# feldroop/floxer

Hardware: NVIDIA B200
Metric: pex_verification_gcups (higher is better)
Workload: dtype u32

## Files before the change

floxer_b200/csrc/dp_kernels.cuh:

```cuda
#pragma once

#include <cstdint>
#include <cuda_runtime.h>

namespace fxg {

constexpr int kNumSymbols = 6;
constexpr int kPeqFrontPadWords = 64;
constexpr int kPeqBackPadWords = 66;
constexpr uint32_t kFlagReverse = 1u;
constexpr uint32_t kFlagInlineRef = 2u;
constexpr int32_t kNoScore = 0x3fffffff;
constexpr int32_t kPoisonScore = 0x7ffffff0;
constexpr uint32_t kWinChunks = 8;
constexpr uint32_t kWinBytes = 2 * kWinChunks * 32;

struct DpTask {
    uint64_t ref_base;
    uint64_t query_base;
    uint64_t trace_base;
    uint32_t n;
    uint32_t m;
    int32_t dlo, dhi;
    uint32_t flags;
// ... 344 lines not shown
        for (uint32_t c = r; c < fill; c += G) load_window_chunk(packed, store_chunks, first_chunk, reverse, c, win);
        uint32_t const n_words = nb * W;
        for (uint32_t w = r; w < n_words; w += G) {
            int32_t const virt = int32_t(pad) - int32_t(32 * w);
            uint32_t const wild = virt >= 32 ? 0xffffffffu : (virt > 0 ? ((1u << virt) - 1u) : 0u);
            uint32_t* const dst = peq + (w / W) * (kNumSymbols * W) + (w % W);
#pragma unroll
            for (int s = 0; s < kNumSymbols; ++s) {
                const uint32_t* plane = L.peq_table + uint64_t(s) * L.peq_plane_words;
                uint32_t x;
                if (!reverse) {
                    x = peq_window(plane, int64_t(T.query_base) - int64_t(pad) + int64_t(32 * w));
                } else {
                    int64_t const y = int64_t(T.query_base) + int64_t(T.m) - 1 + int64_t(pad) - int64_t(32 * w);
                    x = __brev(peq_window(plane, y - 31));
                }
                dst[s * W] = x | wild;
            }
        }
    }
    __syncwarp();

    uint32_t const last_block = nb - 1;
    uint32_t const ck_per_block = ck_records_per_block(int64_t(T.dhi) - int64_t(T.dlo) + 1, ROWS);
    LaneState<W> S;
    S.acc_hp = 0; S.acc_hn = 0; S.ckp = nullptr;
#pragma unroll
    for (int i = 0; i < W; ++i) { S.Pv[i] = 0; S.Mv[i] = 0; }
    S.b = r; S.o_hp = 0x80000000u; S.o_hn = 0;
    S.score = 0; S.best = kNoScore; S.best_col = 0;
    S.eqb = peq;
    int32_t ce_up = 0;
    auto set_block = [&](uint32_t blk) {
        S.cs = 0x7fffffff; S.ce = -1;
        if (!have_task || blk >= nb) return;
        {
            int32_t const hi_up = int32_t(ROWS) * int32_t(blk) + dhi;
            ce_up = hi_up > int32_t(T.n) ? int32_t(T.n) : hi_up;
        }
        int32_t const lo = int32_t(ROWS) * int32_t(blk) + 1 + dlo;
        int32_t const hi = int32_t(ROWS) * int32_t(blk + 1) + dhi;
        int32_t const cs = lo < 1 ? 1 : lo;
        int32_t const ce = hi > int32_t(T.n) ? int32_t(T.n) : hi;
        if (cs <= ce) { S.cs = cs; S.ce = ce; }
    };
    set_block(S.b);
    uint32_t const src_lane = in_ring ? slot * G + (r + G - 1) % G : lane;

    uint32_t const my_end = __reduce_max_sync(0xffffffffu, have_task ? (T.n + nb - 1) : 0u);
    constexpr uint32_t kNever = 0x7fffffffu;

    auto flush_boundary_bits = [&](uint32_t t) {
        uint32_t const left_over = (t - 1) & 31u;
        if (left_over) {
            uint32_t const hb = __brev(S.acc_hp) >> (32 - left_over), nbits = __brev(S.acc_hn) >> (32 - left_over);
            if constexpr (W == 1) *reinterpret_cast<uint2*>(S.ckp + 2) = make_uint2(hb, nbits);
            else *reinterpret_cast<uint4*>(S.ckp + 2 * W) = make_uint4(hb, nbits, 0u, 0u);
        }
    };

    uint32_t my_refill = 0;
    uint32_t t = 1;
    while (t <= my_end) {
        uint32_t const r_hp = __shfl_sync(0xffffffffu, S.o_hp, src_lane);
        uint32_t const r_hn = __shfl_sync(0xffffffffu, S.o_hn, src_lane);
        int32_t const r_sc = __shfl_sync(0xffffffffu, S.score, src_lane);
        if (S.ce >= 0 && int32_t(t) - int32_t(S.b) > S.ce) {
            if (CKPT) flush_boundary_bits(t);
            S.b += G; set_block(S.b);
        }
        int32_t const j = int32_t(t) - int32_t(S.b);
        if (j == S.cs) {
#pragma unroll
            for (int i = 0; i < W; ++i) { S.Pv[i] = 0xffffffffu; S.Mv[i] = 0; }
            if (S.b == 0) {
#pragma unroll
                for (int i = 0; i < W; ++i) {
                    int32_t const virt = int32_t(pad) - 32 * i;
                    S.Pv[i] = virt >= 32 ? 0u : (virt > 0 ? (0xffffffffu << virt) : 0xffffffffu);
                }
                S.score = int32_t(ROWS) - int32_t(pad);
            } else if (S.cs - 1 == ce_up) {
                S.score = r_sc + ROWS;
            } else {
                S.score = r_sc - int32_t(r_hp >> 31) + int32_t(r_hn >> 31) + ROWS;
            }
            S.eqb = peq + S.b * (kNumSymbols * W);
            if (CKPT) {
                S.acc_hp = 0xffffffffu; S.acc_hn = 0;
                S.ckp = L.trace + T.trace_base + uint64_t(S.b) * ck_per_block * ck_record_words(W);
            }
        }
        bool const active = j >= S.cs && j <= S.ce && !dead;
        if (__any_sync(0xffffffffu, t >= my_refill)) {
            my_refill = kNever;
            uint32_t new_base = c_base;
            uint32_t i_hi = 0;
            bool reading = false;
            if (have_task && !dead) {
                int32_t const ti = int32_t(t);
                int32_t const e1 = ti - int32_t(T.n);
                int32_t const e2n = ti - dhi - ROWS;
                int32_t const e2 = e2n > 0 ? (e2n + ROWS) / (ROWS + 1) : 0;
                int32_t const b_top = e1 > e2 ? e1 : e2;
                int32_t const s1 = ti - 1 - dlo;
                int32_t b_low = s1 > 0 ? s1 / (ROWS + 1) : 0;
                if (b_low > ti - 1) b_low = ti - 1;
                if (b_low > int32_t(last_block)) b_low = int32_t(last_block);
                reading = b_top <= int32_t(last_block);
                if (reading) {
                    i_hi = uint32_t(int32_t(phase) + ti + 1 - b_top);
                    if (i_hi >= 32 * (c_base + kWinChunks)) {
                        int32_t const lo = ti - 3 - b_low;
                        new_base = uint32_t(int32_t(phase) + (lo > 0 ? lo : 0)) >> 5;
                        if (new_base <= c_base || i_hi >= 32 * (new_base + kWinChunks)) { dead = true; new_base = c_base; }
                    }
                }
            }
            uint32_t const rounds = __reduce_max_sync(0xffffffffu, (new_base - c_base + G - 1) / G);
            for (uint32_t k = 0; k < rounds; ++k) {
                uint32_t const c = c_base + kWinChunks + r + k * G;
                if (c < new_base + kWinChunks) load_window_chunk(packed, store_chunks, first_chunk, reverse, c, win);
            }
            c_base = new_base;
            if (reading && !dead) my_refill = t + (32 * (c_base + kWinChunks) - i_hi);
        }
        __syncwarp();
        uint8_t const* const win0 = win + phase - 32 * kWinChunks * (c_base / kWinChunks);
        uint32_t my_evt = active ? uint32_t(S.ce) + S.b + 1u : (S.cs == 0x7fffffff ? kNever : uint32_t(S.cs) + S.b);
        my_evt = min(my_evt, my_refill);
        auto upper_at = [&](uint32_t step) {
            if (S.b == 0) return Upper{0u, 0u};
            return int32_t(step) - int32_t(S.b) > ce_up ? Upper{0u, 0x80000000u} : Upper{1u, 0u};
        };
        Upper const up_first = upper_at(t), up_rest = upper_at(t + 1);
        bool const peel = __any_sync(0xffffffffu, up_first.keep != up_rest.keep);
        if (active && S.b > 0 && int32_t(t) - int32_t(S.b) < ce_up) my_evt = min(my_evt, uint32_t(ce_up) + S.b);
        uint32_t const evt = min(__reduce_min_sync(0xffffffffu, my_evt), my_end + 1);
        bool const any_last = __any_sync(0xffffffffu, active && S.b == last_block);
        if (any_last) run_steps<W, CKPT, true>(S, t, evt, active, src_lane, last_block, win0, win, L.two, up_first, up_rest, peel);
        else run_steps<W, CKPT, false>(S, t, evt, active, src_lane, last_block, win0, win, L.two, up_first, up_rest, peel);
        t = evt;
    }
    if (CKPT && S.ce >= 0 && int32_t(t) - int32_t(S.b) > S.ce) flush_boundary_bits(t);
    uint32_t const owner = last_block % G;
    if (have_task && r == owner) {
        DpResult res; res.score = dead ? kPoisonScore : S.best; res.end_col = S.best_col;
        L.results[T.out] = res;
    }
}

__host__ __device__ constexpr int dp_min_ctas(int W) { return W <= 2 ? 28 : (W == 4 ? 25 : (W == 8 ? 19 : (W == 16 ? 14 : 8))); }
template <int W, bool CKPT>
__global__ void __launch_bounds__(32, dp_min_ctas(W)) dp_kernel(DpLaunch const L) {
    extern __shared__ __align__(16) uint8_t smem[];
    uint32_t const tasks_per_warp = 32u / L.group;
    uint32_t const n_tasks = L.n_tasks_dev ? __ldg(L.n_tasks_dev) : L.n_tasks;
    const DpTask* tasks = L.tasks;
    if (L.class_active) { for (uint32_t c = 0; c < L.cls; ++c) tasks += __ldg(L.class_active + c); }
    for (uint32_t g = blockIdx.x; g * tasks_per_warp < n_tasks; g += gridDim.x) {
        dp_task_group<W, CKPT>(L, tasks, g, n_tasks, smem);
        __syncwarp();
    }
}

constexpr uint32_t kWideThreads = 128;
constexpr uint32_t kWideG = 64;
__host__ __device__ constexpr size_t wide_smem_bytes() { return size_t(kNumSymbols) * 32 * kWideThreads * 4 + 2 * kWideThreads * 16; }

template <bool CKPT>
__global__ void __launch_bounds__(kWideThreads, 1) dp_wide_kernel(DpLaunch const L) {
    extern __shared__ __align__(16) uint8_t smem[];
    constexpr int W = 32;
    constexpr int ROWS = 32 * W;
    uint32_t* const eq_all = reinterpret_cast<uint32_t*>(smem);
    uint4* const pub = reinterpret_cast<uint4*>(smem + size_t(kNumSymbols) * 32 * kWideThreads * 4);
    uint32_t const l = threadIdx.x;
    uint32_t const n_tasks = L.n_tasks_dev ? __ldg(L.n_tasks_dev) : L.n_tasks;
    const DpTask* tasks = L.tasks;
    if (L.class_active) { for (uint32_t c = 0; c < L.cls; ++c) tasks += __ldg(L.class_active + c); }
    for (uint32_t task_id = blockIdx.x; task_id < n_tasks; task_id += gridDim.x) {
        DpTask const T = tasks[task_id];
        uint32_t const nb = (T.m + ROWS - 1) / ROWS;
        uint32_t const pad = nb * ROWS - T.m;
        int32_t const dlo = T.dlo - int32_t(pad), dhi = T.dhi - int32_t(pad);
        bool const reverse = (T.flags & kFlagReverse) != 0;
        const uint32_t* const packed = (T.flags & kFlagInlineRef) ? L.inline_packed : L.ref_packed;
        bool const have = l < nb;
        int32_t cs = 0x7fffffff, ce = -1;
        if (have) {
            int32_t const lo = int32_t(ROWS) * int32_t(l) + 1 + dlo, hi = int32_t(ROWS) * int32_t(l + 1) + dhi;
            int32_t const a = lo < 1 ? 1 : lo, b = hi > int32_t(T.n) ? int32_t(T.n) : hi;
            if (a <= b) { cs = a; ce = b; }
        }
        if (have) {
            for (int w = 0; w < W; ++w) {
                uint32_t const gw = l * W + uint32_t(w);
                int32_t const virt = int32_t(pad) - int32_t(32 * gw);
                uint32_t const wild = virt >= 32 ? 0xffffffffu : (virt > 0 ? ((1u << virt) - 1u) : 0u);
                for (int sym = 0; sym < kNumSymbols; ++sym) {
                    const uint32_t* plane = L.peq_table + uint64_t(sym) * L.peq_plane_words;
                    uint32_t x;
                    if (!reverse) x = peq_window(plane, int64_t(T.query_base) - int64_t(pad) + int64_t(32 * gw));
                    else x = __brev(peq_window(plane, int64_t(T.query_base) + int64_t(T.m) - 1 + int64_t(pad) - int64_t(32 * gw) - 31));
                    eq_all[(uint32_t(sym) * 32 + uint32_t(w)) * kWideThreads + l] = x | wild;
                }
            }
        }
        uint32_t Pv[W], Mv[W];
#pragma unroll
        for (int i = 0; i < W; ++i) { Pv[i] = 0; Mv[i] = 0; }
        int32_t score = 0, best = kNoScore;
        uint32_t best_col = 0;
        uint32_t acc_hp = 0xffffffffu, acc_hn = 0;
        uint32_t const ck_per_block = ck_records_per_block(int64_t(T.dhi) - int64_t(T.dlo) + 1, ROWS);
        uint32_t* ckp = CKPT ? L.trace + T.trace_base + uint64_t(l) * ck_per_block * ck_record_words(W) : nullptr;
        pub[l] = make_uint4(0x80000000u, 0u, 0u, 0u);
        pub[kWideThreads + l] = make_uint4(0x80000000u, 0u, 0u, 0u);
        __syncthreads();
        uint32_t const t_end = T.n + nb - 1;
        bool const is_last = have && l == nb - 1;
        for (uint32_t t = 1; t <= t_end; ++t) {
            int32_t const j = int32_t(t) - int32_t(l);
            uint4 const up = l > 0 ? pub[((t - 1) & 1u) * kWideThreads + l - 1] : make_uint4(0u, 0u, 0u, 0u);
            bool const active = have && j >= cs && j <= ce;
            uint4 mine = make_uint4(0x80000000u, 0u, uint32_t(score), 0u);
            if (active) {
                if (j == cs) {
#pragma unroll
                    for (int i = 0; i < W; ++i) { Pv[i] = 0xffffffffu; Mv[i] = 0; }
                    if (l == 0) {
#pragma unroll
                        for (int i = 0; i < W; ++i) {
                            int32_t const virt = int32_t(pad) - 32 * i;
                            Pv[i] = virt >= 32 ? 0u : (virt > 0 ? (0xffffffffu << virt) : 0xffffffffu);
                        }
                        score = int32_t(ROWS) - int32_t(pad);
                    } else if (cs - 1 == (int32_t(ROWS) * int32_t(l) + dhi > int32_t(T.n) ? int32_t(T.n) : int32_t(ROWS) * int32_t(l) + dhi)) {
                        score = int32_t(up.z) + ROWS;
                    } else {
                        score = int32_t(up.z) - int32_t(up.x >> 31) + int32_t(up.y >> 31) + ROWS;
                    }
                    acc_hp = 0xffffffffu; acc_hn = 0;
                }
                uint64_t const pos = reverse ? T.ref_base + uint64_t(T.n) - uint64_t(j) : T.ref_base + uint64_t(j) - 1;
                uint32_t c = packed_base(packed, pos);
                if (c >= uint32_t(kNumSymbols)) c = 0;
                uint32_t Eq[W];
#pragma unroll
                for (int w = 0; w < W; ++w) Eq[w] = eq_all[(c * 32 + uint32_t(w)) * kWideThreads + l];
                uint32_t hp, hn, no_hp[1];
                block_column<W, false>(Pv, Mv, Eq, l == 0 ? 0u : up.x, l == 0 ? 0u : up.y, hp, hn, no_hp);
                score += int32_t(hp >> 31) - int32_t(hn >> 31);
                if (is_last && score <= best) { best = score; best_col = uint32_t(j); }
                mine = make_uint4(hp, hn, uint32_t(score), 0u);
                if (CKPT) {
                    acc_hp = __funnelshift_l(hp, acc_hp, 1); acc_hn = __funnelshift_l(hn, acc_hn, 1);
                    if ((t & 31u) == 0) { write_checkpoint<W>(ckp, Pv, Mv, __brev(acc_hp), __brev(acc_hn)); ckp += ck_record_words(W); }
                    else if (j == ce) {
                        uint32_t const left_over = t & 31u;
                        *reinterpret_cast<uint4*>(ckp + 2 * W) = make_uint4(__brev(acc_hp) >> (32 - left_over), __brev(acc_hn) >> (32 - left_over), 0u, 0u);
                    }
                }
            }
            pub[(t & 1u) * kWideThreads + l] = mine;
            __syncthreads();
        }
        if (is_last) { DpResult res; res.score = best; res.end_col = best_col; L.results[T.out] = res; }
        __syncthreads();
    }
}

struct WalkResult {
    uint32_t begin_col;
    uint32_t cigar_len;
};

struct Walk2Task {
    uint64_t ck_base;
    uint64_t ref_base;
    uint64_t query_base;
    uint64_t cigar_base;
    uint32_t n, m;
    int32_t dlo, dhi;
    uint32_t end_col;
    uint32_t score;
    uint32_t flags;
    uint32_t cigar_cap;
    uint32_t out;
    uint32_t reserved;
};

struct Walk2Launch {
    const Walk2Task* tasks; uint32_t n_tasks;
    const uint32_t* ck;
    const uint32_t* ref_packed; const uint32_t* inline_packed;
    const uint32_t* peq_table; uint64_t peq_plane_words;
    const uint8_t* query_pool;
    uint32_t* cigars;
    WalkResult* results;
    uint32_t two;
};

__host__ __device__ constexpr uint32_t walk2_threads() { return 64u; }
__host__ __device__ constexpr uint32_t walk2_per_cta(uint32_t W) { return walk2_threads() / W; }
__host__ __device__ constexpr uint32_t walk2_words_per_group(uint32_t W) { return 64 * W + 2 + kNumSymbols * W + 8; }
__host__ __device__ constexpr size_t walk2_smem_bytes(uint32_t W) { return size_t(walk2_words_per_group(W)) * walk2_per_cta(W) * 4; }

template <int W>
__global__ void __launch_bounds__(walk2_threads()) walk2_kernel(Walk2Launch const L) {
    extern __shared__ __align__(16) uint32_t w2_smem[];
    constexpr int ROWS = 32 * W;
    constexpr uint32_t RECW = ck_record_words(W);
    constexpr uint32_t PER_CTA = walk2_per_cta(W);
    uint32_t const w = threadIdx.x % W;
    uint32_t const grp = threadIdx.x / W;
    uint32_t* const bits = w2_smem + grp * walk2_words_per_group(W);
    uint32_t* const eq_g = bits + 64 * W + 2;
    uint8_t* const tile_chars = reinterpret_cast<uint8_t*>(eq_g + kNumSymbols * W);
    uint32_t const id = blockIdx.x * PER_CTA + grp;
    bool const mine = id < L.n_tasks;
    bool done = !mine;
    Walk2Task T;
    if (!done) T = L.tasks[id];
    else { T = Walk2Task{}; T.m = 1; }
    const uint32_t* const ref = (T.flags & kFlagInlineRef) ? L.inline_packed : L.ref_packed;
    uint32_t const nb = (T.m + ROWS - 1) / ROWS;
    uint32_t const pad = nb * ROWS - T.m;
    int32_t const dlo = T.dlo - int32_t(pad), dhi = T.dhi - int32_t(pad);
    uint32_t const ck_per_block = ck_records_per_block(int64_t(T.dhi) - int64_t(T.dlo) + 1, ROWS);
    const uint32_t* const ck = L.ck + T.ck_base;
    uint32_t* const slot_end = L.cigars + T.cigar_base + T.cigar_cap;
    bool const writer = w == 0;

    auto block_steps = [&](uint32_t b, int32_t& ts, int32_t& te) {
        int32_t const lo = int32_t(ROWS) * int32_t(b) + 1 + dlo, hi = int32_t(ROWS) * int32_t(b + 1) + dhi;
        ts = (lo < 1 ? 1 : lo) + int32_t(b);
        te = (hi > int32_t(T.n) ? int32_t(T.n) : hi) + int32_t(b);
    };

    uint32_t i = T.m, j = T.end_col;
    uint32_t n_runs = 0, cur_code = 0, cur_len = 0, errors = 0;
    bool bad = false;
    uint32_t eq_block = 0xffffffffu;
    auto flush_run = [&]() {
        if (cur_len) {
            if (n_runs < T.cigar_cap) { if (writer) slot_end[-1 - int64_t(n_runs)] = (cur_len << 4) | ((0x2187u >> (4 * cur_code)) & 15u); }
            else bad = true;
            ++n_runs;
        }
    };
    auto emit = [&](uint32_t code, uint32_t len) {
        if (code == cur_code) { cur_len += len; return; }
        flush_run();
        cur_code = code; cur_len = len;
    };

    struct TileIn { uint32_t raw[5]; uint32_t sh; uint32_t pv, mv; uint32_t hpA, hnA, hpB, hnB; };
    TileIn X;
    bool pf_valid = false; uint32_t pf_b = 0, pf_q = 0;
    auto fetch_tile = [&](uint32_t b, uint32_t q, TileIn& Y) {
        int32_t ts, te; block_steps(b, ts, te);
        int32_t const t0 = 32 * int32_t(q - 1);
        int64_t const pos0 = int64_t(T.ref_base) + int64_t(t0) - int64_t(b);
        int64_t const w0 = pos0 >= 0 ? (pos0 >> 3) : -((7 - pos0) >> 3);
        Y.sh = uint32_t(pos0 - w0 * 8) * 4;
#pragma unroll
        for (int k = 0; k < 5; ++k) Y.raw[k] = w0 + k >= 0 ? __ldg(ref + (w0 + k)) : 0u;
        Y.pv = 0; Y.mv = 0;
        if (t0 >= ts) {
            const uint32_t* rec = ck + (uint64_t(b) * ck_per_block + uint32_t(int32_t(q - 1) - ((ts + 31) >> 5))) * RECW;
            Y.pv = rec[w]; Y.mv = rec[W + w];
        }
        Y.hpA = 0xffffffffu; Y.hnA = 0; Y.hpB = 0xffffffffu; Y.hnB = 0;
        if (b > 0) {
            int32_t us, ue; block_steps(b - 1, us, ue);
            int32_t const uq_first = (us + 31) >> 5, uq_last = (ue + 31) >> 5;
            const uint32_t* const urec = ck + uint64_t(b - 1) * ck_per_block * RECW;
            constexpr int BO = W == 1 ? 2 : 2 * W;
            if (int32_t(q) >= uq_first && int32_t(q) <= uq_last) { uint2 const v = *reinterpret_cast<const uint2*>(urec + uint64_t(int32_t(q) - uq_first) * RECW + BO); Y.hpA = v.x; Y.hnA = v.y; }
            if (int32_t(q) - 1 >= uq_first && int32_t(q) - 1 <= uq_last) { uint2 const v = *reinterpret_cast<const uint2*>(urec + uint64_t(int32_t(q) - 1 - uq_first) * RECW + BO); Y.hpB = v.x; Y.hnB = v.y; }
        }
    };

    while (!__all_sync(0xffffffffu, done)) {
        uint32_t b = 0, q = 0;
        if (!done) {
            if (i == 0) done = true;
            else if (j == 0) { emit(2, i); errors += i; i = 0; done = true; }
        }
        uint32_t Pv1[1] = {0}, Mv1[1] = {0};
        uint32_t top_hp = 0, top_hn = 0;
        int32_t p_first = 0, n_steps = 0;
        uint32_t wi0 = 0;
        if (!done) {
            uint32_t const u = i + pad;
            b = (u - 1) / ROWS;
            wi0 = ((u - 1) % ROWS) >> 5;
            uint32_t const t_cell = j + b;
            q = (t_cell + 31) >> 5;
            int32_t ts, te; block_steps(b, ts, te);
            int32_t const t0 = 32 * int32_t(q - 1);
            int32_t const t_lo = t0 + 1 > ts ? t0 + 1 : ts, t_hi = int32_t(t_cell) < te ? int32_t(t_cell) : te;
            p_first = t_lo - t0 - 1; n_steps = t_hi - t_lo + 1;
            if (n_steps < 0) n_steps = 0;
            if (!(pf_valid && pf_b == b && pf_q == q)) fetch_tile(b, q, X);
            pf_valid = false;
#pragma unroll
            for (int k = 0; k < 4; ++k) {
                if (uint32_t(k) % uint32_t(W) == w % 4u) {
                    uint32_t lo8, hi8;
                    unpack8(__funnelshift_r(X.raw[k], X.raw[k + 1], X.sh), lo8, hi8);
                    *reinterpret_cast<uint2*>(tile_chars + 8 * k) = make_uint2(lo8, hi8);
                }
            }
            if (t0 >= ts) { Pv1[0] = X.pv; Mv1[0] = X.mv; }
            else {
                int32_t const virt = b == 0 ? int32_t(pad) - 32 * int32_t(w) : 0;
                Pv1[0] = virt >= 32 ? 0u : (virt > 0 ? (0xffffffffu << virt) : 0xffffffffu);
                Mv1[0] = 0;
            }
            if (b > 0) {
                int32_t us, ue; block_steps(b - 1, us, ue);
                top_hp = (X.hpA << 1) | (X.hpB >> 31);
                top_hn = (X.hnA << 1) | (X.hnB >> 31);
                int32_t const p_lo = us - t0, p_hi = ue - t0;
                uint32_t valid = 0;
                if (p_hi >= 0 && p_lo <= 31) {
                    uint32_t const lo = p_lo > 0 ? uint32_t(p_lo) : 0u, hi = p_hi < 31 ? uint32_t(p_hi) : 31u;
                    valid = (hi == 31 ? 0xffffffffu : ((1u << (hi + 1)) - 1u)) & ~((1u << lo) - 1u);
                }
                top_hp = (top_hp & valid) | ~valid;
                top_hn &= valid;
            }
            if (eq_block != b) {
                eq_block = b;
                uint32_t const gw = b * W + w;
                int32_t const virt = int32_t(pad) - int32_t(32 * gw);
                uint32_t const wild = virt >= 32 ? 0xffffffffu : (virt > 0 ? ((1u << virt) - 1u) : 0u);
#pragma unroll
                for (int sym = 0; sym < kNumSymbols; ++sym) {
                    const uint32_t* plane = L.peq_table + uint64_t(sym) * L.peq_plane_words;
                    eq_g[sym * W + w] = peq_window(plane, int64_t(T.query_base) - int64_t(pad) + int64_t(32 * gw)) | wild;
                }
            }
        }
        __syncwarp();
        {
            int32_t const my_last = (!done && w <= wi0) ? n_steps - 1 + int32_t(wi0) : -1;
            int32_t const t_max = __reduce_max_sync(0xffffffffu, my_last);
            uint32_t out_hp = 0, out_hn = 0;
            bool const works = !done && w <= wi0;
            auto eq_of = [&](int32_t sidx) -> uint32_t {
                int32_t const p = p_first + (sidx < 0 ? 0 : sidx);
                return eq_g[uint32_t(tile_chars[p > 31 ? 31 : p]) * W + w];
            };
            uint32_t eq_next = works ? eq_of(-int32_t(w)) : 0u;
            for (int32_t tau = 0; tau <= t_max; ++tau) {
                uint32_t in_hp = __shfl_up_sync(0xffffffffu, out_hp, 1, W);
                uint32_t in_hn = __shfl_up_sync(0xffffffffu, out_hn, 1, W);
                int32_t const sidx = tau - int32_t(w);
                if (works && sidx >= 0 && sidx < n_steps) {
                    uint32_t const p = uint32_t(p_first + sidx);
                    if (w == 0) { in_hp = ((top_hp >> p) & 1u) << 31; in_hn = ((top_hn >> p) & 1u) << 31; }
                    uint32_t Eq1[1], hp_all[1];
                    Eq1[0] = eq_next;
                    eq_next = eq_of(sidx + 1);
                    block_column<1, true>(Pv1, Mv1, Eq1, in_hp, in_hn, out_hp, out_hn, hp_all);
                    uint32_t const hp = hp_all[0], vp = Pv1[0];
                    uint32_t const low = hp | ~(vp | Eq1[0]);
                    uint32_t const high = hp | vp;
                    *reinterpret_cast<uint2*>(bits + (p * W + w) * 2) = make_uint2(low, high);
                }
            }
        }
        __syncwarp();
        if (!done) {
            int32_t ts, te; block_steps(b, ts, te);
            if (q >= 2 && 32 * int32_t(q - 1) >= ts) { fetch_tile(b, q - 1, X); pf_valid = true; pf_b = b; pf_q = q - 1; }
        }
        if (!done) {
            uint32_t const u0 = i + pad;
            int32_t p = int32_t(j + b) - 32 * int32_t(q - 1) - 1;
            int32_t r = int32_t((u0 - 1) % ROWS);
            int32_t const r_min = b == 0 ? int32_t(pad) : 0;
            int32_t const p_min = (int32_t(b) + 1 - 32 * int32_t(q - 1) - 1) > 0 ? (int32_t(b) + 1 - 32 * int32_t(q - 1) - 1) : 0;
            uint32_t ops_err = 0;
            while (p >= p_min && r >= r_min) {
                uint2 const v = *reinterpret_cast<const uint2*>(bits + (uint32_t(p) * W + (uint32_t(r) >> 5)) * 2);
                uint32_t const bit = uint32_t(r) & 31u;
                uint32_t const lo1 = (v.x >> bit) & 1u, hi1 = (v.y >> bit) & 1u;
                uint32_t const code = lo1 | (hi1 << 1);
                p -= int32_t(code != 2u);
                r -= int32_t(code != 3u);
                ops_err += code != 0u;
                if (code == cur_code) ++cur_len;
                else { flush_run(); cur_code = code; cur_len = 1; }
            }
            int32_t const p0 = int32_t(j + b) - 32 * int32_t(q - 1) - 1, r0 = int32_t((u0 - 1) % ROWS);
            j -= uint32_t(p0 - p); i -= uint32_t(r0 - r);
            errors += ops_err;
        }
        __syncwarp();
    }
    if (mine && writer) {
        flush_run();
        if (errors != T.score) bad = true;
        WalkResult R; R.begin_col = j; R.cigar_len = bad ? 0xffffffffu : n_runs;
        L.results[T.out] = R;
    }
}

struct NodeRec {
    uint32_t from, m, k;
    uint16_t parent;
    uint8_t depth;
    uint8_t cls;
};
struct LeafRec { uint32_t from; uint32_t parent; };
struct AnchorRec16 { uint64_t reference_position; uint32_t pex_leaf_index; uint32_t reference_id; };
struct ReadRec {
    uint32_t walk_begin;
    uint32_t n_forward;
    uint32_t node_base, leaf_base;
    uint64_t qoff_forward, qoff_reverse;
    uint32_t root_from, root_m, root_k;
    uint32_t root_extra;
    uint32_t member;
    uint32_t n_walks;
    uint32_t reserved0, reserved1;
};
struct WalkRec {
    int64_t diag;
    uint64_t qoff;
    uint32_t node;
    uint32_t node_base;
    uint32_t ref_id;
    uint32_t orient;
};
constexpr uint32_t kDeadNode = 0xffffffffu;
constexpr uint32_t kAtRootNode = 0xfffffffeu;
constexpr uint32_t kNoParent = 0xffffffffu;
constexpr int kWalkBits = 28;
constexpr uint32_t kMaxDeviceWalks = 1u << kWalkBits;
constexpr unsigned long long kWalkMask = (1ull << kWalkBits) - 1;
constexpr int kMaxLevelClasses = 32;

__global__ void gather_reads_kernel(const ReadRec* __restrict__ src, ReadRec* __restrict__ dst, uint32_t n, uint32_t walk0, uint32_t node0,
                                    uint32_t leaf0, uint64_t pool_shift, uint32_t member) {
    uint32_t const i = blockIdx.x * blockDim.x + threadIdx.x;
    if (i >= n) return;
    ReadRec r = src[i];
    r.walk_begin += walk0; r.node_base += node0; r.leaf_base += leaf0;
    r.qoff_forward += pool_shift; r.qoff_reverse += pool_shift; r.member = member;
    dst[i] = r;
}

__device__ __forceinline__ uint32_t read_of_walk(const ReadRec* __restrict__ reads, uint32_t n_reads, uint32_t i) {
    uint32_t lo = 0, hi = n_reads;
    while (hi - lo > 1) { uint32_t const mid = (lo + hi) >> 1; if (reads[mid].walk_begin <= i) lo = mid; else hi = mid; }
    return lo;
}

__global__ void walk_init_kernel(const AnchorRec16* __restrict__ anchors, const ReadRec* __restrict__ reads, uint32_t n_reads,
                                 const LeafRec* __restrict__ leaves, WalkRec* __restrict__ walks, uint32_t* __restrict__ node, uint32_t n_walks,
                                 uint32_t direct) {
    uint32_t const i = blockIdx.x * blockDim.x + threadIdx.x;
    if (i >= n_walks) return;
    ReadRec const R = reads[read_of_walk(reads, n_reads, i)];
    AnchorRec16 const A = anchors[i];
    LeafRec const L = leaves[R.leaf_base + A.pex_leaf_index];
    uint32_t const orient = i - R.walk_begin >= R.n_forward ? 1u : 0u;
    WalkRec w;
    w.diag = int64_t(A.reference_position) - int64_t(L.from);
    w.qoff = orient ? R.qoff_reverse : R.qoff_forward;
    w.node_base = R.node_base; w.ref_id = A.reference_id; w.orient = orient;
    w.node = (!direct && L.parent != kNoParent && L.parent != 0) ? R.node_base + L.parent : kAtRootNode;
    walks[i] = w;
    node[i] = w.node;
}

struct LevelCtx {
    const WalkRec* walks; const NodeRec* nodes; uint32_t n_walks;
    const uint64_t* ref_base; const uint64_t* ref_len;
    uint32_t* node;
    uint64_t* ask_ws; uint32_t* ask_len; uint8_t* flag;
    unsigned long long* rep;
    unsigned long long* rep_min;
    uint32_t* n_inner; uint64_t* sum_inner; uint64_t* cells_inner;
    DpTask* tasks;
    uint32_t* counts;
    uint32_t* class_active;
    const DpResult* results;
    unsigned long long* totals;
    uint32_t level, infer;
    uint8_t cls_W[kMaxLevelClasses];
};
enum : uint8_t { kWalkActive = 1, kWalkComputed = 2, kWalkYes = 4, kWalkAsksLeftmost = 8 };

__device__ __forceinline__ uint32_t class_offset(const uint32_t* __restrict__ class_active, uint32_t cls) {
    uint32_t o = 0;
    for (uint32_t c = 0; c < cls; ++c) o += class_active[c];
    return o;
}

__device__ __forceinline__ void warp_add(unsigned long long* addr, unsigned long long v) {
    unsigned const active = __activemask();
    unsigned const lo = __reduce_add_sync(active, unsigned(v & 0xffffffu)), hi = __reduce_add_sync(active, unsigned(v >> 24));
    if ((threadIdx.x & 31u) == unsigned(__ffs(int(active)) - 1)) atomicAdd(addr, (unsigned long long)lo + ((unsigned long long)hi << 24));
}
__device__ __forceinline__ void warp_add_keyed(unsigned long long* base, uint32_t stride, uint32_t key, unsigned long long v) {
    unsigned const active = __activemask();
    unsigned const peers = __match_any_sync(active, key);
    unsigned const lo = __reduce_add_sync(peers, unsigned(v & 0xffffffu)), hi = __reduce_add_sync(peers, unsigned(v >> 24));
    if ((threadIdx.x & 31u) == unsigned(__ffs(int(peers)) - 1)) atomicAdd(base + size_t(key) * stride, (unsigned long long)lo + ((unsigned long long)hi << 24));
}
__device__ __forceinline__ uint32_t warp_slot(uint32_t* counters, uint32_t key) {
    unsigned const active = __activemask();
    unsigned const peers = __match_any_sync(active, key);
    unsigned const lane = threadIdx.x & 31u;
    int const leader = __ffs(int(peers)) - 1;
    uint32_t base = 0;
    if (int(lane) == leader) base = atomicAdd(counters + key, uint32_t(__popc(peers)));
    base = __shfl_sync(peers, base, leader);
    return base + uint32_t(__popc(peers & ((1u << lane) - 1u)));
}

__device__ __forceinline__ void emit_level_task(LevelCtx const& C, uint32_t i, NodeRec const& N, uint64_t qoff) {
    uint32_t const slot = class_offset(C.class_active, N.cls) + warp_slot(C.counts, N.cls);
    DpTask t;
    t.ref_base = C.ask_ws[i]; t.query_base = qoff + N.from; t.trace_base = 0;
    t.n = C.ask_len[i]; t.m = N.m; t.dlo = -int32_t(N.k); t.dhi = int32_t(t.n) - int32_t(N.m) + int32_t(N.k);
    t.flags = 0; t.out = i;
    C.tasks[slot] = t;
    uint32_t const W = C.cls_W[N.cls], rows = 32 * W, nb = W ? (N.m + rows - 1) / rows : 0;
    int64_t const pad = int64_t(nb) * rows - N.m;
    unsigned long long ws = 0;
    for (uint32_t b = 0; b < nb; ++b) {
        int64_t lo = int64_t(rows) * b + 1 + t.dlo - pad, hi = int64_t(rows) * (b + 1) + t.dhi - pad;
        if (lo < 1) lo = 1;
        if (hi > int64_t(t.n)) hi = t.n;
        if (hi >= lo) ws += (unsigned long long)(hi - lo + 1) * W;
    }
    warp_add(C.totals, 1ull);
    warp_add(C.totals + 1, ws);
}

__global__ void level_begin_kernel(LevelCtx const C) {
    uint32_t const i = blockIdx.x * blockDim.x + threadIdx.x;
    uint8_t f = 0;
    uint32_t cls = 0xffu;
    if (i < C.n_walks) {
        uint32_t const nd = C.node[i];
        if (nd < kAtRootNode) {
            NodeRec const N = C.nodes[nd];
            if (N.depth == C.level) {
                WalkRec const Wk = C.walks[i];
                int64_t const s = Wk.diag + int64_t(N.from) - int64_t(N.k);
                uint64_t const offset = s >= 0 ? uint64_t(s) : 0;
                uint64_t const base = uint64_t(N.m) + 2ull * N.k + 1;
                uint64_t const room = C.ref_len[Wk.ref_id] - offset;
                uint64_t const len = base < room ? base : room;
                C.n_inner[i] += 1; C.sum_inner[i] += len; C.cells_inner[i] += uint64_t(N.m) * len;
                if (int64_t(N.m) - int64_t(len) > int64_t(N.k)) {
                    C.node[i] = kDeadNode;
                } else {
                    uint64_t const ws = C.ref_base[Wk.ref_id] + offset;
                    C.ask_ws[i] = ws; C.ask_len[i] = uint32_t(len);
                    f = kWalkActive;
                    cls = N.cls;
                    if (C.infer) {
                        atomicMax(C.rep + (size_t(nd) * 2 + Wk.orient), (unsigned long long)((ws << kWalkBits) | i));
                        atomicMin(C.rep_min + (size_t(nd) * 2 + Wk.orient), (unsigned long long)((ws << kWalkBits) | i));
                    }
                }
            }
        }
        C.flag[i] = f;
    }
    uint32_t const peers = __match_any_sync(0xffffffffu, cls);
    if (cls != 0xffu && (threadIdx.x & 31u) == uint32_t(__ffs(int(peers)) - 1)) atomicAdd(C.class_active + cls, uint32_t(__popc(peers)));
}

__global__ void level_first_kernel(LevelCtx const C) {
    uint32_t const i = blockIdx.x * blockDim.x + threadIdx.x;
    if (i >= C.n_walks || !(C.flag[i] & kWalkActive)) return;
    uint32_t const nd = C.node[i];
    WalkRec const Wk = C.walks[i];
    if (C.infer && uint32_t(C.rep[size_t(nd) * 2 + Wk.orient] & kWalkMask) != i) return;
    emit_level_task(C, i, C.nodes[nd], Wk.qoff);
    C.flag[i] |= kWalkComputed;
}

__global__ void level_second_kernel(LevelCtx const C) {
    uint32_t const i = blockIdx.x * blockDim.x + threadIdx.x;
    if (i >= C.n_walks) return;
    uint8_t const f = C.flag[i];
    if (!(f & kWalkActive) || (f & kWalkComputed)) return;
    uint32_t const nd = C.node[i];
    NodeRec const N = C.nodes[nd];
    WalkRec const Wk = C.walks[i];
    size_t const key = size_t(nd) * 2 + Wk.orient;
    uint32_t const a = uint32_t(C.rep[key] & kWalkMask);
    DpResult const R = C.results[a];
    bool const a_yes = R.score <= int32_t(N.k);
    uint64_t const ws = C.ask_ws[i]; uint32_t const len = C.ask_len[i];
    if (ws == C.ask_ws[a] && len == C.ask_len[a]) { if (a_yes) C.flag[i] = f | kWalkYes; return; }
    bool const same_ref = C.walks[a].ref_id == Wk.ref_id;
    if (a_yes) {
        if (same_ref && ws + len >= C.ask_ws[a] + R.end_col) { C.flag[i] = f | kWalkYes; warp_add(C.totals + 2, 1ull); return; }
    } else if (same_ref) {
        uint32_t const c = uint32_t(C.rep_min[key] & kWalkMask);
        if (C.walks[c].ref_id == Wk.ref_id && C.ask_ws[a] - C.ask_ws[c] <= uint64_t(N.k) + 1) {
            if (i != c) { C.flag[i] = f | kWalkAsksLeftmost; return; }
        }
    }
    emit_level_task(C, i, N, Wk.qoff);
    C.flag[i] = f | kWalkComputed;
}

__global__ void level_third_kernel(LevelCtx const C) {
    uint32_t const i = blockIdx.x * blockDim.x + threadIdx.x;
    if (i >= C.n_walks) return;
    uint8_t const f = C.flag[i];
    if (!(f & kWalkAsksLeftmost)) return;
    uint32_t const nd = C.node[i];
    NodeRec const N = C.nodes[nd];
    WalkRec const Wk = C.walks[i];
    uint32_t const c = uint32_t(C.rep_min[size_t(nd) * 2 + Wk.orient] & kWalkMask);
    DpResult const R = C.results[c];
    if (R.score > int32_t(N.k)) { warp_add(C.totals + 2, 1ull); return; }
    uint64_t const ws = C.ask_ws[i]; uint32_t const len = C.ask_len[i];
    uint64_t const end = C.ask_ws[c] + R.end_col;
    if ((ws == C.ask_ws[c] && len == C.ask_len[c]) ||
        (end <= ws + len && int64_t(end) - int64_t(N.m) - int64_t(R.score) >= int64_t(ws))) {
        C.flag[i] = f | kWalkYes; warp_add(C.totals + 2, 1ull); return;
    }
    emit_level_task(C, i, N, Wk.qoff);
    C.flag[i] = f | kWalkComputed;
}

__global__ void level_advance_kernel(LevelCtx const C) {
    uint32_t const i = blockIdx.x * blockDim.x + threadIdx.x;
    if (i >= C.n_walks) return;
    uint8_t const f = C.flag[i];
    if (!(f & kWalkActive)) return;
    uint32_t const nd = C.node[i];
    NodeRec const N = C.nodes[nd];
    bool const yes = (f & kWalkComputed) ? C.results[i].score <= int32_t(N.k) : (f & kWalkYes) != 0;
    C.node[i] = yes ? C.walks[i].node_base + N.parent : kDeadNode;
}

struct DecideCtx {
    const WalkRec* walks; const uint32_t* node; const ReadRec* reads; uint32_t n_reads;
    const uint64_t* ref_len;
    const uint32_t* n_inner; const uint64_t* sum_inner; const uint64_t* cells_inner;
    uint8_t* root_flag;
    uint32_t* root_count;
    uint32_t* inserted;
    unsigned long long* member_totals;
    uint32_t ivopt;
};
constexpr int kMemberTotals = 8;

__device__ __forceinline__ void root_window(ReadRec const& R, int64_t diag, uint64_t ref_len, uint64_t& start, uint64_t& len) {
    uint64_t const base = uint64_t(R.root_m) + 2ull * R.root_k + 1;
    int64_t const s = diag + int64_t(R.root_from) - int64_t(R.root_k) - int64_t(R.root_extra);
    start = s >= 0 ? uint64_t(s) : 0;
    uint64_t const full = base + 2ull * R.root_extra, room = ref_len - start;
    len = full < room ? full : room;
}

__global__ void decide_kernel(DecideCtx const C) {
    uint32_t const lane = threadIdx.x & 31u;
    uint32_t const pair = (blockIdx.x * blockDim.x + threadIdx.x) >> 5;
    if (pair >= 2 * C.n_reads) return;
    ReadRec const R = C.reads[pair >> 1];
    uint32_t const orient = pair & 1u;
    uint32_t const w0 = R.walk_begin + (orient ? R.n_forward : 0u);
    uint32_t const w1 = orient ? R.walk_begin + R.n_walks : R.walk_begin + R.n_forward;
    uint32_t n_ins = 0, n_root = 0;
    uint32_t ins_ref = 0; uint64_t ins_start = 0, ins_end = 0;
    unsigned long long s_n = 0, s_sum = 0, s_cells = 0, s_av = 0, s_avsum = 0;
    for (uint32_t base = w0; base < w1; base += 32) {
        uint32_t const i = base + lane;
        bool const have = i < w1;
        uint32_t ref = 0; uint64_t rs = 0, len = 0; bool reached = false;
        if (have) {
            WalkRec const Wk = C.walks[i];
            ref = Wk.ref_id;
            root_window(R, Wk.diag, C.ref_len[ref], rs, len);
            reached = C.node[i] != kDeadNode;
        }
        uint64_t const re = rs + len;
        uint64_t const e0 = R.root_extra > re ? 0 : re - R.root_extra;
        uint64_t const te = e0 > rs + 1 ? e0 : rs + 1;
        uint64_t const ts = te - 1 < rs + R.root_extra ? te - 1 : rs + R.root_extra;
        bool my_avoided = false, my_root = false;
        uint32_t const n_here = min(32u, w1 - base);
        for (uint32_t q = 0; q < n_here; ++q) {
            uint32_t const q_ref = __shfl_sync(0xffffffffu, ref, q);
            uint64_t const q_rs = __shfl_sync(0xffffffffu, rs, q), q_re = __shfl_sync(0xffffffffu, re, q);
            uint64_t const q_ts = __shfl_sync(0xffffffffu, ts, q), q_te = __shfl_sync(0xffffffffu, te, q);
            bool const q_reached = __shfl_sync(0xffffffffu, int(reached), q) != 0;
            bool avoided = false;
            if (C.ivopt) {
                bool hit = lane < min(n_ins, 32u) && ins_ref == q_ref && ins_start <= q_ts && ins_end >= q_te;
                for (uint32_t e = 32 + lane; e < n_ins; e += 32) {
                    WalkRec const Wi = C.walks[C.inserted[w0 + e]];
                    uint64_t is, il;
                    root_window(R, Wi.diag, C.ref_len[Wi.ref_id], is, il);
                    hit |= Wi.ref_id == q_ref && is <= q_ts && is + il >= q_te;
                }
// ... 170 lines not shown
```

Before: 665,500.

## Run traceback walk one task per thread with cp.async Peq staging and batched match skipping

Reworks the walk2 traceback kernel so each thread handles a whole task instead of W cooperating lanes. Each thread recomputes the full W-word block column itself, stores only a window of up to four words of traceback bit-planes in shared memory, and prefetches the next block's Peq words with cp.async. The traceback loop now reads up to eight diagonal cells per iteration and skips runs of matches with ffs. This removes warp shuffles, syncwarps and lockstep idling across tasks, at the cost of more registers per thread, more shared memory per thread, and redundant computation of the W-word column.

```diff
diff --git a/floxer_b200/csrc/dp_kernels.cuh b/floxer_b200/csrc/dp_kernels.cuh
--- a/floxer_b200/csrc/dp_kernels.cuh
+++ b/floxer_b200/csrc/dp_kernels.cuh
@@ -670,28 +670,28 @@
     uint32_t two;
 };
 
-__host__ __device__ constexpr uint32_t walk2_threads() { return 64u; }
-__host__ __device__ constexpr uint32_t walk2_per_cta(uint32_t W) { return walk2_threads() / W; }
-__host__ __device__ constexpr uint32_t walk2_words_per_group(uint32_t W) { return 64 * W + 2 + kNumSymbols * W + 8; }
-__host__ __device__ constexpr size_t walk2_smem_bytes(uint32_t W) { return size_t(walk2_words_per_group(W)) * walk2_per_cta(W) * 4; }
+__host__ __device__ constexpr uint32_t walk2_threads() { return 32u; }
+__host__ __device__ constexpr uint32_t walk2_per_cta(uint32_t) { return walk2_threads(); }
+__host__ __device__ constexpr uint32_t walk2_win_words(uint32_t W) { return W < 4 ? W : 4; }
+__host__ __device__ constexpr size_t walk2_smem_bytes(uint32_t W) {
+    return size_t(walk2_threads()) * (32 * walk2_win_words(W) * 8 + kNumSymbols * (2 * W + 1) * 4);
+}
 
 template <int W>
 __global__ void __launch_bounds__(walk2_threads()) walk2_kernel(Walk2Launch const L) {
     extern __shared__ __align__(16) uint32_t w2_smem[];
     constexpr int ROWS = 32 * W;
     constexpr uint32_t RECW = ck_record_words(W);
-    constexpr uint32_t PER_CTA = walk2_per_cta(W);
-    uint32_t const w = threadIdx.x % W;
-    uint32_t const grp = threadIdx.x / W;
-    uint32_t* const bits = w2_smem + grp * walk2_words_per_group(W);
-    uint32_t* const eq_g = bits + 64 * W + 2;
-    uint8_t* const tile_chars = reinterpret_cast<uint8_t*>(eq_g + kNumSymbols * W);
-    uint32_t const id = blockIdx.x * PER_CTA + grp;
-    bool const mine = id < L.n_tasks;
-    bool done = !mine;
-    Walk2Task T;
-    if (!done) T = L.tasks[id];
-    else { T = Walk2Task{}; T.m = 1; }
+    constexpr int NW = int(walk2_win_words(W));
+    constexpr int NG = W / NW;
+    constexpr uint32_t N = walk2_threads();
+    uint32_t const lane = threadIdx.x;
+    uint2* const planes = reinterpret_cast<uint2*>(w2_smem) + lane;
+    uint32_t* const eq = w2_smem + 2 * 32 * NW * N + lane;
+    uint32_t* const stage = eq + kNumSymbols * W * N;
+    uint32_t const id = blockIdx.x * N + lane;
+    if (id >= L.n_tasks) return;
+    Walk2Task const T = L.tasks[id];
     const uint32_t* const ref = (T.flags & kFlagInlineRef) ? L.inline_packed : L.ref_packed;
     uint32_t const nb = (T.m + ROWS - 1) / ROWS;
     uint32_t const pad = nb * ROWS - T.m;
@@ -699,7 +699,6 @@
     uint32_t const ck_per_block = ck_records_per_block(int64_t(T.dhi) - int64_t(T.dlo) + 1, ROWS);
     const uint32_t* const ck = L.ck + T.ck_base;
     uint32_t* const slot_end = L.cigars + T.cigar_base + T.cigar_cap;
-    bool const writer = w == 0;
 
     auto block_steps = [&](uint32_t b, int32_t& ts, int32_t& te) {
         int32_t const lo = int32_t(ROWS) * int32_t(b) + 1 + dlo, hi = int32_t(ROWS) * int32_t(b + 1) + dhi;
@@ -711,9 +710,22 @@
     uint32_t n_runs = 0, cur_code = 0, cur_len = 0, errors = 0;
     bool bad = false;
     uint32_t eq_block = 0xffffffffu;
+    uint32_t staged = 0xffffffffu;
+    auto peq_bit = [&](uint32_t blk) { return int64_t(T.query_base) - int64_t(pad) + int64_t(32 * W) * blk + int64_t(kPeqFrontPadWords) * 32; };
+    auto stage_peq = [&](uint32_t blk) {
+        int64_t const w0 = peq_bit(blk) >> 5;
+#pragma unroll
+        for (int sym = 0; sym < kNumSymbols; ++sym) {
+            const uint32_t* src = L.peq_table + uint64_t(sym) * L.peq_plane_words + w0;
+            for (int x = 0; x <= W; ++x)
+                asm volatile("cp.async.ca.shared.global [%0], [%1], 4;" :: "r"(uint32_t(__cvta_generic_to_shared(stage + (sym * (W + 1) + x) * N))), "l"(src + x) : "memory");
+        }
+        asm volatile("cp.async.commit_group;" ::: "memory");
+        staged = blk;
+    };
     auto flush_run = [&]() {
         if (cur_len) {
-            if (n_runs < T.cigar_cap) { if (writer) slot_end[-1 - int64_t(n_runs)] = (cur_len << 4) | ((0x2187u >> (4 * cur_code)) & 15u); }
+            if (n_runs < T.cigar_cap) slot_end[-1 - int64_t(n_runs)] = (cur_len << 4) | ((0x2187u >> (4 * cur_code)) & 15u);
             else bad = true;
             ++n_runs;
         }
@@ -724,21 +736,32 @@
         cur_code = code; cur_len = len;
     };
 
-    struct TileIn { uint32_t raw[5]; uint32_t sh; uint32_t pv, mv; uint32_t hpA, hnA, hpB, hnB; };
+    struct TileIn { uint32_t raw[5]; uint32_t sh; uint32_t pv[W], mv[W]; uint32_t hpA, hnA, hpB, hnB; };
     TileIn X;
     bool pf_valid = false; uint32_t pf_b = 0, pf_q = 0;
     auto fetch_tile = [&](uint32_t b, uint32_t q, TileIn& Y) {
         int32_t ts, te; block_steps(b, ts, te);
         int32_t const t0 = 32 * int32_t(q - 1);
-        int64_t const pos0 = int64_t(T.ref_base) + int64_t(t0) - int64_t(b);
+        int32_t const t_lo = t0 + 1 > ts ? t0 + 1 : ts;
+        int64_t const pos0 = int64_t(T.ref_base) + int64_t(t_lo) - 1 - int64_t(b);
         int64_t const w0 = pos0 >= 0 ? (pos0 >> 3) : -((7 - pos0) >> 3);
         Y.sh = uint32_t(pos0 - w0 * 8) * 4;
 #pragma unroll
         for (int k = 0; k < 5; ++k) Y.raw[k] = w0 + k >= 0 ? __ldg(ref + (w0 + k)) : 0u;
-        Y.pv = 0; Y.mv = 0;
         if (t0 >= ts) {
             const uint32_t* rec = ck + (uint64_t(b) * ck_per_block + uint32_t(int32_t(q - 1) - ((ts + 31) >> 5))) * RECW;
-            Y.pv = rec[w]; Y.mv = rec[W + w];
+            if constexpr (W % 4 == 0) {
+#pragma unroll
+                for (int x = 0; x < W; x += 4) {
+                    uint4 const a = __ldg(reinterpret_cast<const uint4*>(rec + x)), c = __ldg(reinterpret_cast<const uint4*>(rec + W + x));
+                    Y.pv[x] = a.x; Y.pv[x + 1] = a.y; Y.pv[x + 2] = a.z; Y.pv[x + 3] = a.w;
+                    Y.mv[x] = c.x; Y.mv[x + 1] = c.y; Y.mv[x + 2] = c.z; Y.mv[x + 3] = c.w;
+                }
+            } else {
+                uint4 const a = __ldg(reinterpret_cast<const uint4*>(rec));
+                if constexpr (W == 1) { Y.pv[0] = a.x; Y.mv[0] = a.y; }
+                else { Y.pv[0] = a.x; Y.pv[1] = a.y; Y.mv[0] = a.z; Y.mv[1] = a.w; }
+            }
         }
         Y.hpA = 0xffffffffu; Y.hnA = 0; Y.hpB = 0xffffffffu; Y.hnB = 0;
         if (b > 0) {
@@ -746,137 +769,150 @@
             int32_t const uq_first = (us + 31) >> 5, uq_last = (ue + 31) >> 5;
             const uint32_t* const urec = ck + uint64_t(b - 1) * ck_per_block * RECW;
             constexpr int BO = W == 1 ? 2 : 2 * W;
-            if (int32_t(q) >= uq_first && int32_t(q) <= uq_last) { uint2 const v = *reinterpret_cast<const uint2*>(urec + uint64_t(int32_t(q) - uq_first) * RECW + BO); Y.hpA = v.x; Y.hnA = v.y; }
-            if (int32_t(q) - 1 >= uq_first && int32_t(q) - 1 <= uq_last) { uint2 const v = *reinterpret_cast<const uint2*>(urec + uint64_t(int32_t(q) - 1 - uq_first) * RECW + BO); Y.hpB = v.x; Y.hnB = v.y; }
+            if (int32_t(q) >= uq_first && int32_t(q) <= uq_last) { uint2 const v = __ldg(reinterpret_cast<const uint2*>(urec + uint64_t(int32_t(q) - uq_first) * RECW + BO)); Y.hpA = v.x; Y.hnA = v.y; }
+            if (int32_t(q) - 1 >= uq_first && int32_t(q) - 1 <= uq_last) { uint2 const v = __ldg(reinterpret_cast<const uint2*>(urec + uint64_t(int32_t(q) - 1 - uq_first) * RECW + BO)); Y.hpB = v.x; Y.hnB = v.y; }
         }
     };
 
-    while (!__all_sync(0xffffffffu, done)) {
-        uint32_t b = 0, q = 0;
-        if (!done) {
-            if (i == 0) done = true;
-            else if (j == 0) { emit(2, i); errors += i; i = 0; done = true; }
-        }
-        uint32_t Pv1[1] = {0}, Mv1[1] = {0};
+    while (i != 0) {
+        if (j == 0) { emit(2, i); errors += i; i = 0; break; }
+        uint32_t const u = i + pad;
+        uint32_t const b = (u - 1) / ROWS;
+        int32_t const r0 = int32_t((u - 1) % ROWS);
+        uint32_t const wg = uint32_t(r0 >> 5) / NW;
+        uint32_t const t_cell = j + b;
+        uint32_t const q = (t_cell + 31) >> 5;
+        int32_t ts, te; block_steps(b, ts, te);
+        if (int32_t(t_cell) < ts || int32_t(t_cell) > te) { bad = true; break; }
+        int32_t const t0 = 32 * int32_t(q - 1);
+        int32_t const p_first = (t0 + 1 > ts ? t0 + 1 : ts) - t0 - 1, p_last = int32_t(t_cell) - t0 - 1;
+        int32_t const n_steps = p_last - p_first + 1;
+        if (!(pf_valid && pf_b == b && pf_q == q)) fetch_tile(b, q, X);
+        uint32_t cw[4];
+#pragma unroll
+        for (int k = 0; k < 4; ++k) cw[k] = __funnelshift_r(X.raw[k], X.raw[k + 1], X.sh);
+        uint32_t Pv[W], Mv[W];
+#pragma unroll
+        for (int x = 0; x < W; ++x) {
+            if (t0 >= ts) { Pv[x] = X.pv[x]; Mv[x] = X.mv[x]; }
+            else {
+                int32_t const virt = b == 0 ? int32_t(pad) - 32 * x : 0;
+                Pv[x] = virt >= 32 ? 0u : (virt > 0 ? (0xffffffffu << virt) : 0xffffffffu);
+                Mv[x] = 0;
+            }
+        }
         uint32_t top_hp = 0, top_hn = 0;
-        int32_t p_first = 0, n_steps = 0;
-        uint32_t wi0 = 0;
-        if (!done) {
-            uint32_t const u = i + pad;
-            b = (u - 1) / ROWS;
-            wi0 = ((u - 1) % ROWS) >> 5;
-            uint32_t const t_cell = j + b;
-            q = (t_cell + 31) >> 5;
-            int32_t ts, te; block_steps(b, ts, te);
-            int32_t const t0 = 32 * int32_t(q - 1);
-            int32_t const t_lo = t0 + 1 > ts ? t0 + 1 : ts, t_hi = int32_t(t_cell) < te ? int32_t(t_cell) : te;
-            p_first = t_lo - t0 - 1; n_steps = t_hi - t_lo + 1;
-            if (n_steps < 0) n_steps = 0;
-            if (!(pf_valid && pf_b == b && pf_q == q)) fetch_tile(b, q, X);
-            pf_valid = false;
-#pragma unroll
-            for (int k = 0; k < 4; ++k) {
-                if (uint32_t(k) % uint32_t(W) == w % 4u) {
-                    uint32_t lo8, hi8;
-                    unpack8(__funnelshift_r(X.raw[k], X.raw[k + 1], X.sh), lo8, hi8);
-                    *reinterpret_cast<uint2*>(tile_chars + 8 * k) = make_uint2(lo8, hi8);
+        if (b > 0) {
+            int32_t us, ue; block_steps(b - 1, us, ue);
+            top_hp = (X.hpA << 1) | (X.hpB >> 31);
+            top_hn = (X.hnA << 1) | (X.hnB >> 31);
+            int32_t const p_lo = us - t0, p_hi = ue - t0;
+            uint32_t valid = 0;
+            if (p_hi >= 0 && p_lo <= 31) {
+                uint32_t const lo = p_lo > 0 ? uint32_t(p_lo) : 0u, hi = p_hi < 31 ? uint32_t(p_hi) : 31u;
+                valid = (hi == 31 ? 0xffffffffu : ((1u << (hi + 1)) - 1u)) & ~((1u << lo) - 1u);
+            }
+            top_hp = (top_hp & valid) | ~valid;
+            top_hn &= valid;
+        }
+        if (eq_block != b) {
+            if (staged != b) stage_peq(b);
+            asm volatile("cp.async.wait_all;" ::: "memory");
+            uint32_t const sh = uint32_t(peq_bit(b)) & 31u;
+#pragma unroll 4
+            for (int x = 0; x < W; ++x) {
+                int32_t const virt = int32_t(pad) - int32_t(32 * (b * W + uint32_t(x)));
+                uint32_t const wild = virt >= 32 ? 0xffffffffu : (virt > 0 ? ((1u << virt) - 1u) : 0u);
+#pragma unroll
+                for (int sym = 0; sym < kNumSymbols; ++sym)
+                    eq[(sym * W + x) * N] = __funnelshift_r(stage[(sym * (W + 1) + x) * N], stage[(sym * (W + 1) + x + 1) * N], sh) | wild;
+            }
+            eq_block = b;
+            if (b > 0) stage_peq(b - 1);
+        }
+        {
+            uint32_t nb_ = b, nq = q;
+            if (b > 0 && r0 < p_last - p_first) {
+                int32_t const t_up = int32_t(t_cell) - r0 - 2;
+                int32_t us, ue; block_steps(b - 1, us, ue);
+                if (t_up >= us && t_up <= ue) { nb_ = b - 1; nq = uint32_t(t_up + 31) >> 5; }
+            }
+            if (nb_ == b && !(q >= 2 && t0 >= ts)) nq = 0;
+            pf_valid = nq != 0;
+            if (pf_valid) { fetch_tile(nb_, nq, X); pf_b = nb_; pf_q = nq; }
+        }
+        {
+            uint32_t EqN[W];
+#pragma unroll
+            for (int x = 0; x < W; ++x) EqN[x] = eq[((cw[0] & 15u) * W + x) * N];
+            for (int32_t g = 0; 8 * g < n_steps; ++g) {
+                uint32_t const cg = g == 0 ? cw[0] : (g == 1 ? cw[1] : (g == 2 ? cw[2] : cw[3]));
+                uint32_t const cg1 = g == 0 ? cw[1] : (g == 1 ? cw[2] : cw[3]);
+                int32_t const pg = p_first + 8 * g;
+                uint32_t const thg = top_hp >> pg, tng = top_hn >> pg;
+#pragma unroll
+                for (int s = 0; s < 8; ++s) {
+                    if (8 * g + s >= n_steps) break;
+                    uint32_t Eq[W];
+#pragma unroll
+                    for (int x = 0; x < W; ++x) Eq[x] = EqN[x];
+                    uint32_t const cn = (s < 7 ? (cg >> (4 * (s + 1))) : cg1) & 15u;
+#pragma unroll
+                    for (int x = 0; x < W; ++x) EqN[x] = eq[(cn * W + x) * N];
+                    uint32_t hp_all[W], ohp, ohn;
+                    block_column<W, true>(Pv, Mv, Eq, thg << (31 - s), tng << (31 - s), ohp, ohn, hp_all);
+                    uint2* const dst = planes + (pg + s) * (NW * N);
+#pragma unroll
+                    for (int k = 0; k < NW; ++k) {
+                        uint32_t hp = hp_all[k], vp = Pv[k], e = Eq[k];
+#pragma unroll
+                        for (int gg = 1; gg < NG; ++gg)
+                            if (wg == uint32_t(gg)) { hp = hp_all[gg * NW + k]; vp = Pv[gg * NW + k]; e = Eq[gg * NW + k]; }
+                        dst[k * N] = make_uint2(lop3<0xF1>(hp, vp, e), hp | vp);
+                    }
                 }
             }
-            if (t0 >= ts) { Pv1[0] = X.pv; Mv1[0] = X.mv; }
-            else {
-                int32_t const virt = b == 0 ? int32_t(pad) - 32 * int32_t(w) : 0;
-                Pv1[0] = virt >= 32 ? 0u : (virt > 0 ? (0xffffffffu << virt) : 0xffffffffu);
-                Mv1[0] = 0;
-            }
-            if (b > 0) {
-                int32_t us, ue; block_steps(b - 1, us, ue);
-                top_hp = (X.hpA << 1) | (X.hpB >> 31);
-                top_hn = (X.hnA << 1) | (X.hnB >> 31);
-                int32_t const p_lo = us - t0, p_hi = ue - t0;
-                uint32_t valid = 0;
-                if (p_hi >= 0 && p_lo <= 31) {
-                    uint32_t const lo = p_lo > 0 ? uint32_t(p_lo) : 0u, hi = p_hi < 31 ? uint32_t(p_hi) : 31u;
-                    valid = (hi == 31 ? 0xffffffffu : ((1u << (hi + 1)) - 1u)) & ~((1u << lo) - 1u);
+        }
+        {
+            int32_t p = p_last, r = r0;
+            int32_t const r_lo = max(b == 0 ? int32_t(pad) : 0, int32_t(wg * NW * 32));
+            auto cell = [&](int32_t pp, int32_t rr) { return planes[(pp * NW + (rr >> 5) - int32_t(wg * NW)) * int32_t(N)]; };
+            uint32_t ops_err = 0;
+            while (p >= p_first && r >= r_lo) {
+                int32_t const d_max = min(p - p_first, r - r_lo);
+                int32_t const nv = d_max < 7 ? d_max + 1 : 8;
+                uint32_t m_lo = 0, m_hi = 0;
+#pragma unroll
+                for (int k = 0; k < 8; ++k) {
+                    int32_t const kk = k < nv ? k : 0;
+                    uint2 const v = cell(p - kk, r - kk);
+                    uint32_t const bit = uint32_t(r - kk) & 31u;
+                    m_lo |= ((v.x >> bit) & 1u) << k;
+                    m_hi |= ((v.y >> bit) & 1u) << k;
                 }
-                top_hp = (top_hp & valid) | ~valid;
-                top_hn &= valid;
-            }
-            if (eq_block != b) {
-                eq_block = b;
-                uint32_t const gw = b * W + w;
-                int32_t const virt = int32_t(pad) - int32_t(32 * gw);
-                uint32_t const wild = virt >= 32 ? 0xffffffffu : (virt > 0 ? ((1u << virt) - 1u) : 0u);
-#pragma unroll
-                for (int sym = 0; sym < kNumSymbols; ++sym) {
-                    const uint32_t* plane = L.peq_table + uint64_t(sym) * L.peq_plane_words;
-                    eq_g[sym * W + w] = peq_window(plane, int64_t(T.query_base) - int64_t(pad) + int64_t(32 * gw)) | wild;
+                uint32_t const n0 = __ffs((m_lo | m_hi | (0xffffffffu << nv)) | 0x100u) - 1u;
+                if (n0) {
+                    if (cur_code != 0u) { flush_run(); cur_code = 0; cur_len = 0; }
+                    cur_len += n0; p -= int32_t(n0); r -= int32_t(n0);
                 }
-            }
-        }
-        __syncwarp();
-        {
-            int32_t const my_last = (!done && w <= wi0) ? n_steps - 1 + int32_t(wi0) : -1;
-            int32_t const t_max = __reduce_max_sync(0xffffffffu, my_last);
-            uint32_t out_hp = 0, out_hn = 0;
-            bool const works = !done && w <= wi0;
-            auto eq_of = [&](int32_t sidx) -> uint32_t {
-                int32_t const p = p_first + (sidx < 0 ? 0 : sidx);
-                return eq_g[uint32_t(tile_chars[p > 31 ? 31 : p]) * W + w];
-            };
-            uint32_t eq_next = works ? eq_of(-int32_t(w)) : 0u;
-            for (int32_t tau = 0; tau <= t_max; ++tau) {
-                uint32_t in_hp = __shfl_up_sync(0xffffffffu, out_hp, 1, W);
-                uint32_t in_hn = __shfl_up_sync(0xffffffffu, out_hn, 1, W);
-                int32_t const sidx = tau - int32_t(w);
-                if (works && sidx >= 0 && sidx < n_steps) {
-                    uint32_t const p = uint32_t(p_first + sidx);
-                    if (w == 0) { in_hp = ((top_hp >> p) & 1u) << 31; in_hn = ((top_hn >> p) & 1u) << 31; }
-                    uint32_t Eq1[1], hp_all[1];
-                    Eq1[0] = eq_next;
-                    eq_next = eq_of(sidx + 1);
-                    block_column<1, true>(Pv1, Mv1, Eq1, in_hp, in_hn, out_hp, out_hn, hp_all);
-                    uint32_t const hp = hp_all[0], vp = Pv1[0];
-                    uint32_t const low = hp | ~(vp | Eq1[0]);
-                    uint32_t const high = hp | vp;
-                    *reinterpret_cast<uint2*>(bits + (p * W + w) * 2) = make_uint2(low, high);
+                if (int32_t(n0) < nv) {
+                    uint32_t const code = ((m_lo >> n0) & 1u) | (((m_hi >> n0) & 1u) << 1);
+                    p -= int32_t(code != 2u);
+                    r -= int32_t(code != 3u);
+                    ++ops_err;
+                    if (code == cur_code) ++cur_len;
+                    else { flush_run(); cur_code = code; cur_len = 1; }
                 }
             }
-        }
-        __syncwarp();
-        if (!done) {
-            int32_t ts, te; block_steps(b, ts, te);
-            if (q >= 2 && 32 * int32_t(q - 1) >= ts) { fetch_tile(b, q - 1, X); pf_valid = true; pf_b = b; pf_q = q - 1; }
-        }
-        if (!done) {
-            uint32_t const u0 = i + pad;
-            int32_t p = int32_t(j + b) - 32 * int32_t(q - 1) - 1;
-            int32_t r = int32_t((u0 - 1) % ROWS);
-            int32_t const r_min = b == 0 ? int32_t(pad) : 0;
-            int32_t const p_min = (int32_t(b) + 1 - 32 * int32_t(q - 1) - 1) > 0 ? (int32_t(b) + 1 - 32 * int32_t(q - 1) - 1) : 0;
-            uint32_t ops_err = 0;
-            while (p >= p_min && r >= r_min) {
-                uint2 const v = *reinterpret_cast<const uint2*>(bits + (uint32_t(p) * W + (uint32_t(r) >> 5)) * 2);
-                uint32_t const bit = uint32_t(r) & 31u;
-                uint32_t const lo1 = (v.x >> bit) & 1u, hi1 = (v.y >> bit) & 1u;
-                uint32_t const code = lo1 | (hi1 << 1);
-                p -= int32_t(code != 2u);
-                r -= int32_t(code != 3u);
-                ops_err += code != 0u;
-                if (code == cur_code) ++cur_len;
-                else { flush_run(); cur_code = code; cur_len = 1; }
-            }
-            int32_t const p0 = int32_t(j + b) - 32 * int32_t(q - 1) - 1, r0 = int32_t((u0 - 1) % ROWS);
-            j -= uint32_t(p0 - p); i -= uint32_t(r0 - r);
+            j -= uint32_t(p_last - p); i -= uint32_t(r0 - r);
             errors += ops_err;
         }
-        __syncwarp();
-    }
-    if (mine && writer) {
-        flush_run();
-        if (errors != T.score) bad = true;
-        WalkResult R; R.begin_col = j; R.cigar_len = bad ? 0xffffffffu : n_runs;
-        L.results[T.out] = R;
-    }
+    }
+    asm volatile("cp.async.wait_all;" ::: "memory");
+    flush_run();
+    if (errors != T.score) bad = true;
+    WalkResult R; R.begin_col = j; R.cigar_len = bad ? 0xffffffffu : n_runs;
+    L.results[T.out] = R;
 }
 
 struct NodeRec {
```

Result: no change. 667,900, median of 6 (+0.4%).
